# GadGadGad/Convolutional-KAN-for-Image-Classification

Measured on AMD Instinct MI355X. Metric: images/sec fwd+bwd KAN-VGG11 3x32x32 bs=256/GPU, higher is better.
Workload: dtype f32

## Files before the change

### convolutional-kan-for-image-classification_amd/csrc/kan_internal.h

```cpp
#pragma once
#include <type_traits>
#include "kanconv.h"

int kan_fail_msg(const char* fmt, const char* a);
int kan_raise_lds_limit(const void* kernel, int bytes);

enum : int {
    FAST_GENERIC = 0,
    FAST_BSPLINE_SILU = 1,
    FAST_BSPLINE_GELU = 2,
    FAST_RBF8 = 3,
    FAST_CHEBY5 = 4,
    FAST_CHEBY4 = 5,
    FAST_POLY4 = 6,
    FAST_POLY3 = 7,
    FAST_RBF5 = 8,
    FAST_RELU8 = 9,
    FAST_GRAM4 = 10,
    FAST_POLY1 = 11,
    FAST_LAST = 11
};
enum : unsigned {
    ON_TAP_MAJOR = 1u << 0,
    ON_BIG_TILES = 1u << 1,
// ... 22 lines not shown
        case FAST_CHEBY5: return {KAN_BASIS_CHEBY, 5, false, false, false, 16, ON_TAP_MAJOR | ON_BIG_TILES | ON_BAND_FWD | ON_BAND_BWD_WEIGHT};
        case FAST_CHEBY4: return {KAN_BASIS_CHEBY, 4, false, false, false, 16, ON_TAP_MAJOR | ON_HALO_FWD | ON_BAND_FWD};
        case FAST_POLY4: return {KAN_BASIS_POLY, 5, true, true, false, 16, ON_TAP_MAJOR | ON_BIG_TILES | ON_HALO_FWD | ON_BAND_FWD};
        case FAST_POLY3: return {KAN_BASIS_POLY, 4, true, true, false, 16, ON_TAP_MAJOR};
        case FAST_POLY1: return {KAN_BASIS_POLY, 2, true, true, false, 16, ON_TAP_MAJOR};
        case FAST_RELU8: return {KAN_BASIS_RELU, 9, true, false, false, 16, ON_HALO_FWD | ON_HALO_BWD_WEIGHT | ON_EXPANDED_FWD | ON_EXPANDED};
        case FAST_GRAM4: return {KAN_BASIS_GRAM, 5, true, false, false, 16, ON_HALO_FWD | ON_HALO_BWD_WEIGHT | ON_EXPANDED};
        default: return {-1, 0, false, true, true, 0, 0};
    }
}
constexpr int fast_kind(int f) { return fast_spec(f).kind; }
constexpr int fast_planes(int f) { return fast_spec(f).planes; }
constexpr bool fast_has(int f, unsigned routes) { return (fast_spec(f).routes & routes) == routes && f != FAST_GENERIC; }

template <int V> using IC = std::integral_constant<int, V>;
template <unsigned ROUTES, int F = 1, class Fn>
bool dispatch_fast(int f, Fn&& fn) {
    if constexpr (F > FAST_LAST) {
        return false;
    } else {
        if constexpr (fast_has(F, ROUTES)) {
            if (f == F) { fn(IC<F>{}); return true; }
        }
        return dispatch_fast<ROUTES, F + 1>(f, fn);
    }
}
template <int V, int... REST, class Fn>
void pick(int v, Fn&& fn) {
    if constexpr (sizeof...(REST) == 0) fn(IC<V>{});
    else if (v == V) fn(IC<V>{});
    else pick<REST...>(v, fn);
}
template <class Fn>
void dispatch_kind(int kind, Fn&& fn) {
    pick<KAN_BASIS_BSPLINE, KAN_BASIS_RBF, KAN_BASIS_POLY, KAN_BASIS_FOURIER, KAN_BASIS_RELU, KAN_BASIS_GRAM, KAN_BASIS_CHEBY>(kind, fn);
}

#define KAN_BAND_MAX_TAPS 128
#define KAN_BAND_MAX_PHASES 16
typedef struct KanBandCfg {
    int ok;
    int fast, P, NG, NPLE, NPS;
    int NGR;
    int WO, MO, WP, TO, TP, NT;
    int tiles_o, tiles_p;
    int n_phase, n_taps, n_steps;
    int HC, span_r, OR0, OC0;
    int cells;
    int slots;
    int TS;
    int lds_bytes, wgs_per_cu;
    int fwd_splits;
    int bw_ok, bw_WR, bw_NI, bw_NT, bw_tiles_o, bw_row_tiles, bw_TPI, bw_ptiles, bw_cells, bw_slots, bw_lds_bytes, bw_splits;
    unsigned short bw_ph_rt0[KAN_BAND_MAX_PHASES + 1];
    unsigned char ph_a[KAN_BAND_MAX_PHASES], ph_b[KAN_BAND_MAX_PHASES];
    short ph_tap0[KAN_BAND_MAX_PHASES + 1];
    unsigned short tap_shift[KAN_BAND_MAX_TAPS];
    unsigned short tap_rt[KAN_BAND_MAX_TAPS];
    short tap_step[KAN_BAND_MAX_TAPS], tap_nt[KAN_BAND_MAX_TAPS];
} KanBandCfg;

void kan_band_cfg(const KanGeom* g, const KanBasis* b, int fast, KanBandCfg* cfg);
int kan_band_bwd_weight_launch(const float* dz, const float* x, const float* xn, float* dwp, const KanGeom* g, const KanBasis* b,
                               const KanBandCfg* cfg, int splits, long long slab_elems, void* stream);
int kan_band_fwd_launch(const float* x, const float* xn, const float* wp, float* z, const KanGeom* g, const KanBasis* b,
                        const KanBandCfg* cfg, int splits, long long slab_elems, void* stream);

constexpr int DW_T = 9;
constexpr int DW_MAX_TP = 96;

enum class Route { TAP_MAJOR, DW, BAND, HALO, EXPANDED };

struct FwdCfg { int TO, TP, tiles_o, tiles_p, chunks, splits, slots; };
struct BdCfg { int CH, tiles_c, tiles_p, n_ob, Opad32, chunks, splits; };
struct BwCfg { int TR, TO, tiles_r, tiles_o, chunks, splits, slots; };
struct BwHaloCfg { int R, nimg, spb, n_bands, tiles_r, tiles_o, splits, bands_per_split; };

struct ConvPlan {
    KanPlan pub;
    int fast;
    Route fwd, bwd_data, bwd_weight;
    bool pm_fwd, pm_bwd_data, pm_bwd_weight;
    bool rowblk_bwd_data;
    bool pmdma_xcd, pm_lpt, pm_xcd;
    FwdCfg fc;
    BdCfg bd;
    BwCfg bw;
    BwHaloCfg bwh;
    KanBandCfg band;
};
int plan_conv(const KanGeom* g, const KanBasis* b, ConvPlan* cp);

int live_taps_out(const KanGeom* g, int hw);
int live_taps_in(const KanGeom* g, int hw);
int live_positions_for_tap(const KanGeom* g, int tap);
int balance_tiles(const int* weight, int n, unsigned short* idx);
```

### convolutional-kan-for-image-classification_amd/csrc/kan_plan.hip

```cpp
#include <hip/hip_runtime.h>
#include <cstdio>
#include <cstdlib>
#include <cstring>
#include "kanconv.h"
#include "kan_device.h"
#include "kan_common.h"
#include "kan_internal.h"

namespace {

int fail(const char* msg) { return kan_fail_msg("%s", msg); }

int check(const KanGeom* g, const KanBasis* b) {
    if (!g || !b) return fail("null geometry/basis");
    if (g->groups < 0 || g->groups > 65535) return fail("groups out of range");
    if (g->B <= 0 || g->C <= 0 || g->O <= 0 || g->H <= 0 || g->W <= 0 || g->Ho <= 0 || g->Wo <= 0) return fail("non-positive dimension");
    if (g->kh <= 0 || g->kw <= 0 || g->sh <= 0 || g->sw <= 0 || g->dh <= 0 || g->dw <= 0 || g->ph < 0 || g->pw < 0) return fail("bad conv parameters");
    if (g->kh > 255 || g->kw > 255 || g->C > 65535) return fail("kernel size / channel count out of supported range");
    if ((g->H + 2 * g->ph - g->dh * (g->kh - 1) - 1) / g->sh + 1 != g->Ho || (g->W + 2 * g->pw - g->dw * (g->kw - 1) - 1) / g->sw + 1 != g->Wo)
        return fail("Ho/Wo inconsistent with H/W, kernel, stride, padding, dilation");
    if ((long long)g->B * g->Ho * g->Wo >= (1ll << 31) || (long long)g->B * g->H * g->W >= (1ll << 31)) return fail("pixel count exceeds int32");
    if ((long long)g->B * g->x_bstride * 4 >= (1ll << 31) || (long long)g->B * g->y_bstride * 4 >= (1ll << 31))
        return fail("activation tensors must be smaller than 2 GiB (32-bit buffer offsets)");
    if (g->x_bstride < (long long)ngroups(g) * g->C * g->H * g->W || g->y_bstride < (long long)ngroups(g) * g->O * g->Ho * g->Wo)
// ... 248 lines not shown
    return n;
}

int balance_tiles(const int* weight, int n, unsigned short* idx) {
    if (n < 2 || n > PERM_MAX) return 0;
    int order[PERM_MAX];
    for (int i = 0; i < n; ++i) order[i] = i;
    for (int i = 1; i < n; ++i) {
        int v = order[i], j = i;
        while (j > 0 && weight[order[j - 1]] < weight[v]) { order[j] = order[j - 1]; --j; }
        order[j] = v;
    }
    for (int r = 0; r < n; ++r) {
        const int depth = r / 8, k = r % 8, bin = (depth & 1) ? 7 - k : k;
        int slot = depth * 8 + bin;
        if (slot >= n) slot = r;
        idx[slot] = (unsigned short)order[r];
    }
    bool seen[PERM_MAX] = {false};
    for (int i = 0; i < n; ++i) { if (idx[i] >= n || seen[idx[i]]) return 0; seen[idx[i]] = true; }
    return n;
}

int plan_conv(const KanGeom* g, const KanBasis* b, ConvPlan* cp) {
    if (int rc = check(g, b)) return rc;
    ConvPlan& c = *cp;
    KanPlan* pl = &c.pub;
    const int T = g->kh * g->kw, G = ngroups(g), f = fast_variant(b);
    c.fast = f;
    const bool pm_shape = pmdma_fwd_shape(g, f);
    c.pm_fwd = want_pix_major(g, b, PM_FWD, pm_shape);
    c.pm_bwd_data = want_pix_major(g, b, PM_BWD_DATA, false);
    const bool want_pm_bw = want_pix_major(g, b, PM_BWD_WEIGHT, false);
    const bool dw = dw_direct(g, b);
    const bool halo = halo_fwd(g, b, f, c.pm_fwd);
    c.band.ok = c.band.bw_ok = 0;
    const bool band = band_fwd(g, b, f, dw, c.pm_fwd, halo, &c.band);
    const bool pmdma_fwd = pm_shape && c.pm_fwd;
    const bool pmdma_bw = pmdma_bwd_weight(g, b, f, want_pm_bw);
    const bool halo_bw = halo_bwd_weight(g, f, pmdma_bw);
    c.pm_bwd_weight = want_pm_bw && !halo_bw;
    const bool band_bw = band && c.band.bw_ok && !want_pm_bw && !tuning_off("KAN_BAND_BW");
    c.rowblk_bwd_data = rowblk_bwd_data(g, f, c.pm_bwd_data);
    c.pmdma_xcd = tuning_on("KAN_PMDMA_XCD");
    c.pm_lpt = !tuning_off("KAN_PM_LPT");
    c.pm_xcd = !tuning_off("KAN_PM_XCD");
    c.fwd = dw ? Route::DW : band ? Route::BAND : halo ? Route::HALO : pmdma_fwd ? Route::EXPANDED : Route::TAP_MAJOR;
    c.bwd_data = dw ? Route::DW : Route::TAP_MAJOR;
    c.bwd_weight = dw ? Route::DW : band_bw ? Route::BAND : halo_bw ? Route::HALO : pmdma_bw ? Route::EXPANDED : Route::TAP_MAJOR;
    pl->P = b->n_basis + (b->act != KAN_ACT_NONE);
    pl->K = g->C * T * pl->P;
    {
        int i18 = 18 / pl->P, i16 = 16 / pl->P;
        if (i18 > 4) i18 = 4;
        if (i16 > 4) i16 = 4;
        const bool use18 = (long long)i18 * pl->P * 16 > (long long)i16 * pl->P * 18;
        pl->KC = use18 ? 18 : 16;
        pl->IPC = use18 ? i18 : i16;
        if (pl->P >= 10 && pl->P <= 12) { pl->KC = 12; pl->IPC = 1; }
        if (halo) { pl->KC = 2 * pl->P; pl->IPC = 2; }
    }
    pl->Kpad = ceil_div(g->C * T, pl->IPC) * pl->KC;
    if (band) { pl->KC = c.band.NPLE; pl->IPC = c.band.NG; pl->Kpad = c.band.n_steps * c.band.NPLE; }
    pl->Opad = round_up(g->O, 64);
    pl->packed_weight_bytes = (long long)G * pl->Kpad * pl->Opad * 4;
    c.bd = bd_cfg(g, *pl);
    pl->bwd_data_weight_bytes = (long long)G * T * c.bd.Opad32 * c.bd.tiles_c * 128 * 4;
    pl->fwd_slab_elems = (long long)g->B * g->y_bstride;
    pl->bwd_data_slab_elems = (long long)g->B * g->x_bstride;
    pl->bwd_weight_slab_elems = (long long)G * pl->K * pl->Opad;
    const bool big = big_tiles(f, *pl);
    c.fc = fwd_cfg(g, *pl, big, c.pm_fwd, halo);
    c.bw = bw_cfg(g, *pl, big, c.pm_bwd_weight);
    if (halo_bw) c.bwh = bw_halo_cfg(g, *pl);
    pl->fwd_splits = band ? c.band.fwd_splits : c.fc.splits;
    pl->bwd_data_splits = c.bd.splits;
    pl->bwd_weight_splits = halo_bw ? c.bwh.splits : c.bw.splits;
    if (band_bw) {
        pl->bwd_weight_splits = c.band.bw_splits;
        pl->bwd_weight_slab_elems = (long long)G * pl->Kpad * pl->Opad;
    }
    pl->fwd_target = pl->bwd_data_target = pl->bwd_weight_target = 0;
    const bool rowblk_fwd = halo && g->H == 4 && g->W == 4 && c.fc.TO == 256;
    if (dw) {
        pl->fwd_splits = pl->bwd_data_splits = 1;
        pl->bwd_weight_splits = dw_weight_chunks(g);
        pl->bwd_data_weight_bytes = pl->packed_weight_bytes;
        c.pm_fwd = c.pm_bwd_data = c.pm_bwd_weight = false;
    }
    if (c.pm_fwd) {
        LiveClass cls[16]; const int plane = g->Ho * g->Wo;
        const long long tiles_per_pos = (long long)ceil_div(g->B, c.fc.TP) * c.fc.tiles_o * G;
        for (int hw = 0; hw < plane; ++hw) cls[hw] = LiveClass{tiles_per_pos, live_taps_out(g, hw) * ceil_div(g->C, pl->IPC)};
        pl->fwd_target = pick_target_steps(cls, plane, 8, 4.0 * g->B * g->O * g->Ho * g->Wo * G, &pl->fwd_splits, c.fc.slots);
    }
    if (c.pm_bwd_weight) {
        LiveClass cw[32];
        const long long tiles_per_tap = (long long)ceil_div((long long)g->C * pl->P, c.bw.TR) * c.bw.tiles_o * G;
        for (int tap = 0; tap < T; ++tap) cw[tap] = LiveClass{tiles_per_tap, live_positions_for_tap(g, tap) * ceil_div(g->B, 16)};
        pl->bwd_weight_target = pick_target_steps(cw, T, 16, 4.0 * pl->K * pl->Opad * G, &pl->bwd_weight_splits, c.bw.slots);
    }
    if (c.pm_bwd_data) {
        LiveClass cls[16]; const int plane = g->H * g->W;
        const long long tiles_per_pos = (long long)ceil_div(g->B, 128) * c.bd.tiles_c * G;
        for (int hw = 0; hw < plane; ++hw) cls[hw] = LiveClass{tiles_per_pos, live_taps_in(g, hw) * c.bd.n_ob};
        pl->bwd_data_target = pick_target_steps(cls, plane, 8, 4.0 * g->B * g->C * g->H * g->W * G, &pl->bwd_data_splits);
    }
    pl->fwd_halo = c.fwd == Route::HALO;
    pl->fwd_band = c.fwd == Route::BAND;
    pl->fwd_expanded = c.fwd == Route::EXPANDED;
    pl->bwd_weight_halo = c.bwd_weight == Route::HALO;
    pl->bwd_weight_band = c.bwd_weight == Route::BAND;
    pl->bwd_weight_expanded = c.bwd_weight == Route::EXPANDED;
    pl->x_pm_wanted = (c.pm_fwd && c.fwd != Route::EXPANDED) || (c.pm_bwd_weight && c.bwd_weight != Route::EXPANDED);
    pl->dz_pm_wanted = c.pm_bwd_data || c.pm_bwd_weight;
    pl->e_pm_wanted = pl->fwd_expanded || pl->bwd_weight_expanded;
    pl->e_pm_elems = pl->e_pm_wanted ? (long long)G * g->C * g->H * g->W * pl->P * g->B + 256 : 0;
    pl->row_blocks = (rowblk_fwd ? 1 : 0) | (c.rowblk_bwd_data ? 2 : 0);
    return 0;
}
```

### convolutional-kan-for-image-classification_amd/csrc/kanconv.hip

```cpp
#include <hip/hip_runtime.h>
#include <cstdio>
#include <cstdlib>
#include <cstring>
#include <cmath>
#include <cstdint>
#include <mutex>
#include <type_traits>
#include <vector>
#include "kanconv.h"
#include "kan_device.h"

#include "kan_common.h"
#include "kan_internal.h"

namespace {


thread_local char g_err[512] = "";
int fail(const char* fmt, const char* a = "") {
    snprintf(g_err, sizeof(g_err), fmt, a);
    return -1;
}
}
int kan_fail_msg(const char* fmt, const char* a) { return fail(fmt, a); }
// ... 328 lines not shown
        }
    };

    f32x16 acc[2][2];
#pragma unroll
    for (int a = 0; a < 2; ++a)
#pragma unroll
        for (int b = 0; b < 2; ++b)
#pragma unroll
            for (int r = 0; r < 16; ++r) acc[a][b][r] = 0.f;

    int ch0 = blk.z * chunks_per_split;
    int ch1 = min(n_chunks, ch0 + chunks_per_split);
    unsigned tapmask = 0xffffffffu;
    if (g.pix_major) {
        tapmask = 0;
        const int hwA = px_tile0 / g.B, hwB = min(px_tile0 + TP - 1, Mtot - 1) / g.B;
        for (int hw = hwA; hw <= hwB; ++hw)
            for (int tap = 0; tap < T; ++tap) tapmask |= (tap_alive_out(g, hw, tap) ? 1u : 0u) << tap;
        auto seg = [&](int tap) { return (tap * g.C + IPC - 1) / IPC; };
        const int L = live_step_count(tapmask, T, n_chunks, seg);
        const int S = min((int)gridDim.z, max(1, (L + chunks_per_split - 1) / chunks_per_split));
        if (blk.z >= S) { ch0 = ch1 = n_chunks; }
        else {
            ch0 = blk.z == 0 ? 0 : live_step_pos(tapmask, T, n_chunks, (int)((long long)L * blk.z / S), seg);
            ch1 = blk.z == S - 1 ? n_chunks : live_step_pos(tapmask, T, n_chunks, (int)((long long)L * (blk.z + 1) / S), seg);
        }
    }
    auto next_live = [&](int ch) -> int {
        if (!g.pix_major) return ch;
        while (ch < ch1) {
            const int tapA = (ch * IPC) / g.C, tapB = min(ch * IPC + IPC - 1, NI - 1) / g.C;
            if (((tapmask >> tapA) | (tapmask >> tapB)) & 1u) return ch;
            ch = max(ch + 1, ((tapB + 1) * g.C) / IPC);
        }
        return ch1;
    };
    int ch = next_live(ch0);
    if (ch < ch1) issue(ch, 0);
    __syncthreads();

    const int ao = w_o * 64 + (lane & 31), bp = w_p * 64 + (lane & 31), kh2 = lane >> 5;
    for (int cur = 0; ch < ch1; cur ^= 1) {
        stage(cur);
        asm volatile("s_waitcnt vmcnt(0)" ::: "memory");
        __syncthreads();
        ch = next_live(ch + 1);
        if (ch < ch1) issue(ch, cur ^ 1);
        const float* cW = sW + cur * (KC * TO);
        const float* cE = sE + cur * (KC * TP);
        const unsigned aw = lds_addr(cW + kh2 * TO + ao), ae = lds_addr(cE + kh2 * TP + bp);
        KAN_MFMA_STEP(KC / 2, aw, TO, ae, TP);
    }

    float* zs = z + (size_t)blk.z * slab_elems;
#pragma unroll
    for (int ni = 0; ni < 2; ++ni) {
        const int px = px_tile0 + w_p * 64 + ni * 32 + (lane & 31);
        if (px >= Mtot) continue;
        int b, hw;
        if (g.pix_major) { hw = px / g.B; b = px - hw * g.B; }
        else { b = px / HoWo; hw = px - b * HoWo; }
        float* zb = zs + (size_t)b * g.ybs + hw;
#pragma unroll
        for (int mi = 0; mi < 2; ++mi) {
#pragma unroll
            for (int r = 0; r < 16; ++r) {
                const int o = o_tile0 + w_o * 64 + mi * 32 + mfma_row(r, lane);
                if (o < g.O) zb[(size_t)o * HoWo] = acc[mi][ni][r];
            }
        }
    }
}

#define LDS_READ4H(r0, r1, r2, r3, addrA, addrB0, addrB1, oA0, oA1, oB)                                                 \
    asm volatile("ds_read_b32 %0, %4 offset:%7\n\tds_read_b32 %1, %4 offset:%8\n\tds_read_b32 %2, %5 offset:%9\n\tds_read_b32 %3, %6 offset:%9" \
                 : "=&v"(r0), "=&v"(r1), "=&v"(r2), "=&v"(r3) : "v"(addrA), "v"(addrB0), "v"(addrB1), "n"(oA0), "n"(oA1), "n"(oB) : "memory")

#define LDS_READ3H(r0, r1, r2, addrA, addrB, oA0, oA1, oB)                                                               \
    asm volatile("ds_read_b32 %0, %3 offset:%5\n\tds_read_b32 %1, %3 offset:%6\n\tds_read_b32 %2, %4 offset:%7"         \
                 : "=&v"(r0), "=&v"(r1), "=&v"(r2) : "v"(addrA), "v"(addrB), "n"(oA0), "n"(oA1), "n"(oB) : "memory")
#define LDS_WAIT3(r0, r1, r2, N) asm volatile("s_waitcnt lgkmcnt(" #N ")" : "+v"(r0), "+v"(r1), "+v"(r2) :: "memory")

template <int FAST, int WO, int W, int R, int NIMG>
__global__ __launch_bounds__(WO * 2 * 64, ((WO > 2 && !(R * W == 16 && NIMG * W == 32)) ? 2 : 4)) void k_conv_fwd_halo(
    const float* __restrict__ x, const float* __restrict__ wp, float* __restrict__ z, DevGeom g, DevBasis bs, int Opad,
    int n_pairs, int pairs_per_split, long long slab_elems, unsigned x_bytes, int tiles_o) {
    constexpr int TO = WO * 64, TP = 128, NT = WO * 2 * 64, NW = WO * 2, P = fast_planes(FAST), KC = 2 * P, T = 9;
    constexpr int KIND = fast_kind(FAST);
    constexpr int HW_ = W + 2, HIMG = (R + 2) * HW_, HALO = NIMG * HIMG;
    constexpr int RPI = 256 / TO, NQ = (KC + RPI - 1) / RPI;
    static_assert(NIMG * R * W == TP && HALO % 2 == 0, "tile shape");
    constexpr bool ROWBLK = (R * W == 16 && NIMG * W == 32 && WO == 4);
    __shared__ __attribute__((aligned(16))) float sW[2 * KC * TO];
    __shared__ float sH[2 * P * HALO];
    __shared__ float sTab[KAN_MAX_TABLE];
    __shared__ float sDump[NT];

    const int tid = threadIdx.x, lane = tid & 63;
    const int wave = __builtin_amdgcn_readfirstlane(tid >> 6);
    const int w_o = ROWBLK ? (wave & 3) : (wave >> 1), w_p = ROWBLK ? (wave >> 2) : (wave & 1);
    const int HoWo = g.Ho * g.Wo, HW = g.H * g.W, Mtot = g.B * HoWo;
    const BlockId blk = xcd_block_order(true);
    const int grp = blk.y / tiles_o;
    const int px_tile0 = blk.x * TP, o_tile0 = (blk.y - grp * tiles_o) * TO;
    x += (size_t)grp * g.C * HW;
    z += (size_t)grp * g.O * HoWo;
    wp += (size_t)grp * n_pairs * (T * KC) * Opad;

    if (tid < KAN_MAX_TABLE) sTab[tid] = bs.tab[tid];
    for (int i = tid; i < 2 * P * HALO; i += NT) sH[i] = 0.f;

    const int b0 = px_tile0 / HoWo, h0 = (px_tile0 - b0 * HoWo) / W;
    constexpr int NCELL = 2 * HALO, CPT = (NCELL + NT - 1) / NT;
    int c_src[CPT], c_dst[CPT], c_ch[CPT]; unsigned c_ok = 0;
#pragma unroll
    for (int k = 0; k < CPT; ++k) {
        const int idx = tid + k * NT;
        const int ch = idx / HALO, cell = idx - ch * HALO;
        const int img = cell / HIMG, rc = cell - img * HIMG, hr = rc / HW_, hc = rc - hr * HW_;
        const int b = b0 + img, h = h0 - 1 + hr, w = hc - 1;
        const bool ok = idx < NCELL && b < g.B && (unsigned)h < (unsigned)g.H && (unsigned)w < (unsigned)W;
        c_src[k] = b * (int)g.xbs + ch * HW + h * W + w;
        c_dst[k] = ch * (P * HALO) + cell;
        c_ch[k] = ch;
        c_ok |= (ok ? 1u : 0u) << k;
    }
    const kan_rsrc x_rs = make_rsrc(x, x_bytes);

    const int kh2 = lane >> 5;
    unsigned vb[2];
#pragma unroll
    for (int q = 0; q < 2; ++q) {
        const int n = w_p * 64 + q * 32 + (lane & 31);
        int img = n / (R * W), rem = n - img * (R * W), row = rem / W, col = rem - row * W;
        if (ROWBLK) { row = n / (NIMG * W); rem = n - row * (NIMG * W); img = rem / W; col = rem - img * W; }
        vb[q] = lds_addr(sH + kh2 * (P * HALO) + img * HIMG + (row + 1) * HW_ + (col + 1));
    }
    const int ao = w_o * 64 + (lane & 31);
    const unsigned wlane = (unsigned)((lane / (TO / 4)) * Opad + (lane % (TO / 4)) * 4) * 4u;
    const int wv = wave;

    auto issue_w = [&](int step, int buf) {
        const char* wsrc = (const char*)(wp + (size_t)step * KC * Opad + o_tile0);
        float* dW = sW + buf * (KC * TO);
#pragma unroll
        for (int j = 0; j < (NQ + NW - 1) / NW; ++j) {
            const int q = j * NW + wv;
            if (q < NQ) {
                if (KC % RPI == 0 || q * RPI + (int)(lane / (TO / 4)) < KC)
                    glds16((const float*)(wsrc + (size_t)q * RPI * Opad * 4 + wlane), dW + q * 256);
            }
        }
    };

    f32x16 acc[2][2];
#pragma unroll
    for (int a = 0; a < 2; ++a)
#pragma unroll
        for (int b = 0; b < 2; ++b)
#pragma unroll
            for (int r = 0; r < 16; ++r) acc[a][b][r] = 0.f;

    const int cp0 = blk.z * pairs_per_split, cp1 = min(n_pairs, cp0 + pairs_per_split);
    int buf = 0;
    float xv[CPT];
    auto load_pair = [&](int cp) {
#pragma unroll
        for (int k = 0; k < CPT; ++k)
            xv[k] = buf_load(x_rs, ((c_ok >> k) & 1u) ? (unsigned)(c_src[k] + 2 * cp * HW) * 4u : KAN_OOB);
    };
    if (cp0 < cp1) { issue_w(cp0 * T, 0); load_pair(cp0); }
    __syncthreads();
    for (int cp = cp0; cp < cp1; ++cp) {
        __syncthreads();
#pragma unroll
        for (int k = 0; k < CPT; ++k)
            if ((c_ok >> k) & 1u) stage_unit<KIND, FAST>(bs, sTab, true, xv[k], xv[k], sH + c_dst[k], HALO, sDump + tid, 2 * cp + c_ch[k]);
#pragma unroll 1
        for (int tap = 0; tap < T; ++tap) {
            asm volatile("s_waitcnt vmcnt(0)" ::: "memory");
            __syncthreads();
            const int nxt = cp * T + tap + 1;
            if (nxt < cp1 * T) issue_w(nxt, buf ^ 1);
            if (tap == 4 && cp + 1 < cp1) load_pair(cp + 1);
            const int r = tap / 3, t = tap - r * 3;
            const unsigned sh = (unsigned)(((r - 1) * HW_ + (t - 1)) * 4);
            const unsigned aw = lds_addr(sW + buf * (KC * TO) + kh2 * TO + ao), ab0 = vb[0] + sh, ab1 = vb[1] + sh;
            float fa[2][2], fb[2][2];
            const int dead = !ROWBLK ? -1 : (r == 0 && w_p == 0) ? 0 : (r == 2 && w_p == 1) ? 1 : -1;
            const bool live0 = dead != 0, live1 = dead != 1;
            LDS_READ4H(fa[0][0], fa[0][1], fb[0][0], fb[0][1], aw, ab0, ab1, 0, 32 * 4, 0);
#pragma unroll
            for (int kk = 0; kk < P; ++kk) {
                const int c_ = kk & 1, n_ = c_ ^ 1;
                if (kk + 1 < P) {
                    LDS_READ4H(fa[n_][0], fa[n_][1], fb[n_][0], fb[n_][1], aw, ab0, ab1, (2 * (kk + 1)) * TO * 4, (2 * (kk + 1)) * TO * 4 + 128,
                               (kk + 1) * HALO * 4);
                    LDS_WAIT4(fa[c_][0], fa[c_][1], fb[c_][0], fb[c_][1], 4);
                } else {
                    LDS_WAIT4(fa[c_][0], fa[c_][1], fb[c_][0], fb[c_][1], 0);
                }
                if (!ROWBLK || live0) {
                    acc[0][0] = MFMA32(fa[c_][0], fb[c_][0], acc[0][0]);
                    acc[1][0] = MFMA32(fa[c_][1], fb[c_][0], acc[1][0]);
                }
                if (!ROWBLK || live1) {
                    acc[0][1] = MFMA32(fa[c_][0], fb[c_][1], acc[0][1]);
                    acc[1][1] = MFMA32(fa[c_][1], fb[c_][1], acc[1][1]);
                }
            }
            buf ^= 1;
        }
    }

    float* zs = z + (size_t)blk.z * slab_elems;
#pragma unroll
    for (int ni = 0; ni < 2; ++ni) {
        int px = px_tile0 + w_p * 64 + ni * 32 + (lane & 31);
        if (ROWBLK) {
            const int l = lane & 31;
            px = px_tile0 + (l >> 2) * (R * W) + (w_p * 2 + ni) * W + (l & 3);
        }
        if (px >= Mtot) continue;
        const int b = px / HoWo, hw = px - b * HoWo;
        float* zb = zs + (size_t)b * g.ybs + hw;
#pragma unroll
        for (int mi = 0; mi < 2; ++mi) {
#pragma unroll
            for (int r = 0; r < 16; ++r) {
                const int o = o_tile0 + w_o * 64 + mi * 32 + mfma_row(r, lane);
                if (o < g.O) zb[(size_t)o * HoWo] = acc[mi][ni][r];
            }
        }
    }
}

template <int M>
__device__ __forceinline__ void wave_reduce_scatter(float (&v)[M], int lane, int& idx, float& tot) {
    int base = 0;
    int m = M;
#pragma unroll
    for (int off = 32; off >= 1; off >>= 1) {
        if (m > 1) {
            const int h = m / 2;
            const bool up = (lane & off) != 0;
#pragma unroll
            for (int i = 0; i < M / 2; ++i) {
                if (i < h) {
                    const float keep = up ? v[h + i] : v[i], send = up ? v[i] : v[h + i];
                    v[i] = keep + __shfl_xor(send, off, 64);
                }
            }
            base += up ? h : 0;
            m = h;
        } else {
            v[0] += __shfl_xor(v[0], off, 64);
        }
    }
    idx = base; tot = v[0];
}

template <int KIND, int FAST, int RB = 0>
__global__ __launch_bounds__(256, 4) void k_conv_bwd_data(
    const float* __restrict__ dz, const float* __restrict__ x, const float* __restrict__ xn, const float* __restrict__ wd,
    float* __restrict__ dx, float* __restrict__ dxn, DevGeom g, DevBasis bs, int CH, int n_ct, int n_ob, int Opad16,
    int n_chunks, int chunks_per_split, long long slab_elems, unsigned dz_bytes, TilePerm perm, float* __restrict__ dpar) {
    constexpr int TP = 128, KD = 16, NT = 256;
    __shared__ __attribute__((aligned(16))) float smem[2 * 2 * KD * 128];
    __shared__ float sTab[KAN_MAX_TABLE];

    const int tid = threadIdx.x, lane = tid & 63;
    const int wave = __builtin_amdgcn_readfirstlane(tid >> 6);
    const int w_r = wave >> 1, w_p = wave & 1;
    const int HoWo = g.Ho * g.Wo, HW = g.H * g.W, P = bs.P;
    const int Min = g.B * HW;
    const BlockId blk = xcd_block_order(false);
    const int grp = blk.y / n_ct;
    const int px_tile0 = (perm.n ? (int)perm.idx[blk.x] : blk.x) * TP, ct = blk.y - grp * n_ct;
    const int ncol = n_ct * 128;
    const int pxl = (wave & 1) * 64 + lane, ol0 = wave >> 1;
    const bool idle_rows = (ct * 2 + w_r) * CH >= g.C;
    {
        const size_t xo = (size_t)grp * g.C * HW;
        x += xo; xn += xo; dx += xo; if (dxn) dxn += xo;
        dz += (size_t)grp * g.O * HoWo * (g.pix_major ? g.B : 1);
        wd += (size_t)grp * (g.kh * g.kw) * Opad16 * ncol;
    }

    if (tid < KAN_MAX_TABLE) sTab[tid] = bs.tab[tid];
    const int my_px = px_tile0 + (RB ? ((pxl >> 2) & 7) * 16 + (pxl >> 5) * 4 + (pxl & 3) : pxl);
    const bool pv = my_px < Min;
    int pb, ph_, pw_;
    {
        int hw;
        if (g.pix_major) { hw = my_px / g.B; pb = my_px - hw * g.B; }
        else { pb = my_px / HW; hw = my_px - pb * HW; }
        ph_ = hw / g.W; pw_ = hw - ph_ * g.W;
    }
// ... 1744 lines not shown
    ConvPlan cp;
    if (plan_conv(g, b, &cp)) return 0;
    if ((long long)g->O * g->C * (b->n_basis + 1) * g->kh * g->kw >= (1ll << 31)) return 0;
    return (!pack_needs_clear(g, cp.pub) && cp.fwd != Route::DW && ngroups(g) == 1) ? 1 : 0;
}

int kan_pack_weights_cached(const float* w_base, const float* w_basis, float* wp, float* wd, const KanGeom* g, const KanBasis* b,
                            unsigned long long* ring, int cur, int force, int sample_stride, void* stream) {
    static_assert(KAN_FP_WORDS == 3 * FP_LANES, "ring size");
    if (!ring || cur < 0 || cur > 2 || sample_stride < 1) return fail("bad fingerprint ring arguments");
    if (!kan_pack_cacheable(g, b)) return fail("cached packing is not offered for this geometry (kan_pack_cacheable)");
    const int hb = b->act != KAN_ACT_NONE;
    if ((hb && !w_base) || !w_basis) return fail("null weight pointer");
    if (((size_t)w_basis & 15) || (hb && ((size_t)w_base & 15))) return fail("cached packing needs 16-byte aligned weight tensors");
    const int T = g->kh * g->kw;
    const long long na = hb ? (long long)g->O * g->C * T : 0, nbs = (long long)g->O * g->C * b->n_basis * T;
    const long long groups4 = ((na + 3) / 4 + (nbs + 3) / 4 + sample_stride - 1) / sample_stride;
    long long blocks = (groups4 + 256 * 8 - 1) / (256 * 8); if (blocks > 4096) blocks = 4096; if (blocks < 1) blocks = 1;
    hipLaunchKernelGGL(k_fingerprint, dim3((unsigned)blocks), dim3(256), 0, (hipStream_t)stream, hb ? w_base : w_basis, (unsigned)na, w_basis,
                       (unsigned)nbs, (unsigned)sample_stride, ring, cur);
    if (int rc = launch_ok("fingerprint")) return rc;
    return pack_weights_impl(w_base, w_basis, wp, wd, g, b, force ? nullptr : ring, cur, stream);
}

int kan_unpack_wgrad(const float* dwp, float* dw_base, float* dw_basis, const KanGeom* g, const KanBasis* b, void* stream) {
    ConvPlan cp;
    if (int rc = plan_conv(g, b, &cp)) return rc;
    const KanPlan& pl = cp.pub;
    const int hb = b->act != KAN_ACT_NONE;
    if ((hb && !dw_base) || !dw_basis || !dwp) return fail("null weight-gradient pointer");
    hipStream_t st = (hipStream_t)stream;
    const int T = g->kh * g->kw, G = ngroups(g);
    const long long dwp_gs = (long long)(pl.bwd_weight_band ? pl.Kpad : pl.K) * pl.Opad;
    PackGeo q = pack_geo(g, b, cp, true);
    int n_slabs = pl.bwd_weight_splits;
    if (n_slabs >= 32) {
        hipLaunchKernelGGL(k_fold_slabs, dim3(ceil_div(pl.bwd_weight_slab_elems, 64)), dim3(256), 0, st, const_cast<float*>(dwp), n_slabs,
                           pl.bwd_weight_slab_elems, pl.bwd_weight_slab_elems);
        n_slabs = 1;
    }
    const int nb_base = hb ? ceil_div(g->C * T, 32) : 0;
    dim3 grid(nb_base + ceil_div(g->C * b->n_basis * T, 32), ceil_div(g->O, 32), G);
    hipLaunchKernelGGL(k_unpack, grid, dim3(256), 0, st, dwp, dw_base, dw_basis, q, nb_base, n_slabs, pl.bwd_weight_slab_elems, dwp_gs);
    return launch_ok("unpack");
}

int kan_position_major(const float* src, float* dst, int B, int Cn, int HW, long long bstride, void* stream) {
    if (!src || !dst || B < 1 || Cn < 1 || HW < 1) return fail("bad position_major arguments");
    dim3 grid(ceil_div((long long)Cn * HW, 32), ceil_div(B, 32));
    hipLaunchKernelGGL(k_position_major, grid, dim3(256), 0, (hipStream_t)stream, src, dst, B, Cn * HW, bstride);
    return launch_ok("position_major");
}

int kan_conv_fwd(const float* x, const float* xn, const float* wp, float* z, const KanGeom* g, const KanBasis* b, const float* x_pm,
                 void* stream) {
    ConvPlan cp;
    if (int rc = plan_conv(g, b, &cp)) return rc;
    const KanPlan& pl = cp.pub;
    if (!x || !xn || !wp || !z) return fail("null tensor pointer");
    if ((b->kind == KAN_BASIS_RELU || b->kind == KAN_BASIS_GRAM) && !b->chan_table) return fail("ReLU / Gram bases need their device parameter table (chan_table)");
    hipStream_t st = (hipStream_t)stream;
    if (cp.fwd == Route::DW) {
        DevGeom dgd = dev_geom(g); DevBasis dbd = dev_basis(b);
        dim3 grid(ceil_div((long long)g->B * g->Ho * g->Wo, 256), ngroups(g));
        dispatch_kind(b->kind, [&](auto kind) {
            hipLaunchKernelGGL((k_dw_fwd<decltype(kind)::value>), grid, dim3(256), 0, st, x, xn, wp, z, dgd, dbd, pl.Opad, pl.IPC, pl.KC, pl.Kpad);
        });
        return launch_ok("dw_fwd");
    }
    if (cp.fwd == Route::BAND) {
        if (x != xn && !fast_spec(cp.fast).xn_fwd) return fail("this basis / activation pair runs on single-input kernels: pass xn == x");
        return kan_band_fwd_launch(x, xn, wp, z, g, b, &cp.band, pl.fwd_splits, pl.fwd_slab_elems, stream);
    }
    const FwdCfg& c = cp.fc;
    if ((long long)c.tiles_o * ngroups(g) > 65535) return fail("groups * output tiles exceed the grid limit");
    const unsigned x_bytes = (unsigned)((long long)g->B * g->x_bstride * 4);
    if (cp.fwd == Route::HALO) {
        if (x != xn) return fail("internal: halo forward kernel needs a single input tensor");
        DevGeom dgh = dev_geom(g); DevBasis dbh = dev_basis(b);
        const int n_pairs = g->C / 2, pps = ceil_div(n_pairs, pl.fwd_splits);
        dim3 gridh(c.tiles_p, c.tiles_o * ngroups(g), pl.fwd_splits);
        dispatch_fast<ON_HALO_FWD>(cp.fast, [&](auto fv) {
            constexpr int F = decltype(fv)::value;
            auto launch = [&](auto wo, auto w, auto r, auto nimg) {
                constexpr int WOV = decltype(wo)::value;
                hipLaunchKernelGGL((k_conv_fwd_halo<F, WOV, decltype(w)::value, decltype(r)::value, decltype(nimg)::value>), gridh, dim3(WOV * 128), 0,
                                   st, x, wp, z, dgh, dbh, pl.Opad, n_pairs, pps, pl.fwd_slab_elems, x_bytes, c.tiles_o);
            };
            auto planes = [&](auto wo) {
                if (g->W == 32) launch(wo, IC<32>{}, IC<4>{}, IC<1>{});
                else if (g->W == 16) launch(wo, IC<16>{}, IC<8>{}, IC<1>{});
                else if (g->W == 8) launch(wo, IC<8>{}, IC<8>{}, IC<2>{});
                else launch(wo, IC<4>{}, IC<4>{}, IC<8>{});
            };
            if constexpr (fast_has(F, ON_BIG_TILES)) {
                if (c.TO == 256) return planes(IC<4>{});
            }
            planes(IC<2>{});
        });
        return launch_ok("conv_fwd_halo");
    }
    DevGeom dg = dev_geom(g);
    dg.pix_major = (x_pm && x == xn && cp.pm_fwd) ? 1 : 0;
    if (dg.pix_major) { x = x_pm; xn = x_pm; }
    DevBasis db = dev_basis(b);
    dim3 grid(c.tiles_p, c.tiles_o * ngroups(g), pl.fwd_splits);
    const int cps = dg.pix_major ? pl.fwd_target : ceil_div(c.chunks, pl.fwd_splits);
    TilePerm perm; perm.n = 0;
    if (dg.pix_major) perm = tile_perm(c.tiles_p, [&](int t) {
        const int hw = (int)(((long long)t * c.TP) / g->B);
        return ceil_div(live_taps_out(g, hw < g->Ho * g->Wo ? hw : 0) * ceil_div(g->C, pl.IPC), cps > 0 ? cps : 1);
    });
    if (x != xn && !fast_spec(cp.fast).xn_fwd)
        return fail("this basis / activation pair runs on single-input kernels: pass xn == x");
    auto launch = [&](auto kind, auto fast, auto wo, auto kc) {
        constexpr int WO = decltype(wo)::value;
        hipLaunchKernelGGL((k_conv_fwd<decltype(kind)::value, decltype(fast)::value, WO, 2, decltype(kc)::value>), grid, dim3(WO * 2 * 64), 0, st,
                           x, xn, wp, z, dg, db, pl.Opad, pl.IPC, c.chunks, cps, pl.fwd_slab_elems, x_bytes, perm, c.tiles_o);
    };
    const bool fast = dispatch_fast<ON_TAP_MAJOR>(cp.fast, [&](auto fv) {
        constexpr int F = decltype(fv)::value;
        if constexpr (fast_has(F, ON_BIG_TILES)) {
            if (c.TO == 256) return launch(IC<fast_kind(F)>{}, fv, IC<4>{}, IC<fast_spec(F).kc>{});
        }
        if (c.TO == 128) launch(IC<fast_kind(F)>{}, fv, IC<2>{}, IC<fast_spec(F).kc>{});
        else launch(IC<fast_kind(F)>{}, fv, IC<1>{}, IC<fast_spec(F).kc>{});
    });
    if (!fast) dispatch_kind(b->kind, [&](auto kind) {
        pick<18, 12, 16>(pl.KC, [&](auto kc) {
            if (c.TO == 128) launch(kind, IC<FAST_GENERIC>{}, IC<2>{}, kc);
            else launch(kind, IC<FAST_GENERIC>{}, IC<1>{}, kc);
        });
    });
    return launch_ok("conv_fwd");
}

static int conv_bwd_data_impl(const float* dz, const float* x, const float* xn, const float* wd, float* dx, float* dxn, float* dpar,
                              const KanGeom* g, const KanBasis* b, const float* dz_pm, void* stream);

int kan_conv_bwd_data(const float* dz, const float* x, const float* xn, const float* wd, float* dx, float* dxn,
                      const KanGeom* g, const KanBasis* b, const float* dz_pm, void* stream) {
    return conv_bwd_data_impl(dz, x, xn, wd, dx, dxn, nullptr, g, b, dz_pm, stream);
}

int kan_conv_bwd_data_params(const float* dz, const float* x, const float* xn, const float* wd, float* dx, float* dxn, float* dparams,
                             const KanGeom* g, const KanBasis* b, const float* dz_pm, void* stream) {
    if (!dparams) return fail("null dparams");
    if (b && b->kind != KAN_BASIS_RELU && b->kind != KAN_BASIS_GRAM) return fail("kan_conv_bwd_data_params: only the ReLU-KAN and GRAM bases accumulate parameter gradients in this launch");
    return conv_bwd_data_impl(dz, x, xn, wd, dx, dxn, dparams, g, b, dz_pm, stream);
}

static int conv_bwd_data_impl(const float* dz, const float* x, const float* xn, const float* wd, float* dx, float* dxn, float* dpar,
                              const KanGeom* g, const KanBasis* b, const float* dz_pm, void* stream) {
    ConvPlan cp;
    if (int rc = plan_conv(g, b, &cp)) return rc;
    const KanPlan& pl = cp.pub;
    if (dpar && cp.bwd_data == Route::DW) return fail("kan_conv_bwd_data_params: depthwise layers take the weight-gradient route");
    if (!dz || !x || !xn || !wd || !dx) return fail("null tensor pointer");
    if ((b->kind == KAN_BASIS_RELU || b->kind == KAN_BASIS_GRAM) && !b->chan_table) return fail("ReLU / Gram bases need their device parameter table (chan_table)");
    if (!dxn && x != xn) return fail("dxn is required when xn != x");
    hipStream_t st = (hipStream_t)stream;
    if (cp.bwd_data == Route::DW) {
        DevGeom dgd = dev_geom(g); DevBasis dbd = dev_basis(b);
        dim3 grid(ceil_div((long long)g->B * g->H * g->W, 256), ngroups(g));
        dispatch_kind(b->kind, [&](auto kind) {
            hipLaunchKernelGGL((k_dw_bwd_data<decltype(kind)::value>), grid, dim3(256), 0, st, dz, x, xn, wd, dx, dxn, dgd, dbd, pl.Opad, pl.IPC, pl.KC, pl.Kpad);
        });
        return launch_ok("dw_bwd_data");
    }
    const BdCfg& c = cp.bd;
    DevGeom dg = dev_geom(g);
    dg.pix_major = (dz_pm && cp.pm_bwd_data) ? 1 : 0;
    if (dg.pix_major) dz = dz_pm;
    DevBasis db = dev_basis(b);
    if ((long long)c.tiles_c * ngroups(g) > 65535) return fail("groups * channel tiles exceed the grid limit");
    dim3 grid(c.tiles_p, c.tiles_c * ngroups(g), pl.bwd_data_splits);
// ... 320 lines not shown
```

### convolutional-kan-for-image-classification_amd/ops.py

```python
from __future__ import annotations

import contextlib
import ctypes as C
import os
import weakref
from collections import OrderedDict
from dataclasses import dataclass
from functools import lru_cache
from typing import List, Optional, Sequence, Tuple

import torch

from . import _lib as L


@dataclass(frozen=True)
class ConvSpec:
    kind: int
    n_basis: int
    order: int
    act: int
    p0: float
    p1: float
    table: Tuple[float, ...]
# ... 41 lines not shown
def _plan_key(spec: ConvSpec, shape, Og: int) -> tuple:
    B, Ct, H, W = shape
    return (spec, B, Ct // spec.groups, H, W, Og, Ct, Og * spec.groups)


def _with_phases(basis: L.KanBasis, phases: Optional[torch.Tensor], mode: int = 0) -> L.KanBasis:
    if phases is None:
        return basis
    b = L.KanBasis.from_buffer_copy(basis)
    b.chan_table, b.order = phases.data_ptr(), mode
    return b


def _ptr(t: Optional[torch.Tensor], offset: int = 0) -> C.c_void_p:
    if t is None:
        return C.c_void_p(0)
    return C.c_void_p(t.data_ptr() + 4 * offset)


def _stream(t: torch.Tensor) -> C.c_void_p:
    return C.c_void_p(torch.cuda.current_stream(t.device).cuda_stream)


def _require(t: torch.Tensor, name: str) -> torch.Tensor:
    if not t.is_cuda:
        raise L.KanConvError(f"{name} is on {t.device}: this path runs only on a ROCm device (MI355X); there is no CPU fallback")
    if t.dtype != torch.float32:
        raise L.KanConvError(f"{name} must be float32, got {t.dtype}")
    return t.contiguous()


def _split_weights(spec: ConvSpec, weights: Sequence[torch.Tensor]):
    G = spec.groups
    if spec.has_base:
        return list(weights[:G]), list(weights[G:2 * G])
    return [None] * G, list(weights[:G])


PROFILE: Optional[list] = None


@dataclass
class KernelSample:
    name: str
    flops: float
    executed: float
    layer: str
    start: "torch.cuda.Event"
    end: "torch.cuda.Event"


def _launch(sample, t: torch.Tensor, fn) -> None:
    name, flops, executed, layer = sample
    if PROFILE is None:
        L.check(fn(), name)
        return
    e0, e1 = torch.cuda.Event(enable_timing=True), torch.cuda.Event(enable_timing=True)
    stream = torch.cuda.current_stream(t.device)
    e0.record(stream)
    L.check(fn(), name)
    e1.record(stream)
    PROFILE.append(KernelSample(name, flops, executed, layer, e0, e1))


def _conv_flops(geom, plan) -> float:
    return 2.0 * geom.B * geom.O * geom.Ho * geom.Wo * geom.C * plan.P * geom.kh * geom.kw * max(1, geom.groups)


@lru_cache(maxsize=256)
def _live_fraction(which: str, H: int, W: int, Ho: int, Wo: int, kh: int, kw: int, sh: int, sw: int, ph: int, pw: int, dh: int, dw: int) -> float:
    live = 0
    for ho in range(Ho):
        for wo in range(Wo):
            for r in range(kh):
                for t in range(kw):
                    hi, wi = ho * sh - ph + r * dh, wo * sw - pw + t * dw
                    live += 0 <= hi < H and 0 <= wi < W
    return live / float(Ho * Wo * kh * kw)


_ROW_BLOCK_BIT = {"fwd": 1, "bwd_data": 2, "bwd_weight": 0}


def _executed_flops(geom, plan, which: str) -> float:
    target = {"fwd": plan.fwd_target, "bwd_data": plan.bwd_data_target, "bwd_weight": plan.bwd_weight_target}[which]
    dense = _conv_flops(geom, plan)
    if target <= 0:
        if plan.row_blocks & _ROW_BLOCK_BIT[which]:
            return dense * (5.0 / 6.0)
        return dense
    g = geom
    return dense * _live_fraction(which, g.H, g.W, g.Ho, g.Wo, g.kh, g.kw, g.sh, g.sw, g.ph, g.pw, g.dh, g.dw)


def _layer_tag(geom) -> str:
    return f"{geom.C * max(1, geom.groups)}->{geom.O * max(1, geom.groups)}@{geom.H}x{geom.W} k{geom.kh}x{geom.kw}"


def _sample(which: str, geom, plan, pm: bool, two: bool = False, expanded: bool = False):
    tile = "128" if plan.Opad % 128 == 0 else "64"
    if which == "bwd_data":
        name = "k_conv_bwd_data"
    elif expanded:
        name = f"k_conv_{which}_pmdma/o{tile}"
    elif plan.fwd_band if which == "fwd" else plan.bwd_weight_band:
        name = f"k_band_{which}/o" + ("128" if plan.Opad % 128 == 0 else "192" if plan.Opad == 192 else "64")
    else:
        halo = plan.fwd_halo if which == "fwd" else (plan.bwd_weight_halo and not two)
        name = f"k_conv_{which}{'_halo' if halo else ''}/o{tile}"
    skips = expanded or pm or bool(plan.row_blocks & _ROW_BLOCK_BIT[which])
    dense = _conv_flops(geom, plan)
    return name, dense, _executed_flops(geom, plan, which) if skips else dense, _layer_tag(geom)


def _position_major(t: torch.Tensor, ch_off: int, Cn: int) -> torch.Tensor:
    B, Ct, H, W = t.shape
    out = torch.empty(Cn * H * W * B, device=t.device, dtype=torch.float32)
    L.check(L.load().kan_position_major(_ptr(t, ch_off * H * W), _ptr(out), B, Cn, H * W, Ct * H * W, _stream(t)), "kan_position_major")
    return out


def _stack(ws: Sequence[Optional[torch.Tensor]]) -> Optional[torch.Tensor]:
    if ws[0] is None:
        return None
    return ws[0].unsqueeze(0) if len(ws) == 1 else torch.stack(list(ws))


_PACKED: "OrderedDict[tuple, PackedWeights]" = OrderedDict()
_PACK_CACHE_MAX = int(os.environ.get("KAN_PACK_CACHE", "256"))
_PACK_CACHE_BYTES = int(os.environ.get("KAN_PACK_CACHE_BYTES", str(16 << 30)))
_PACK_SAMPLE = max(1, int(os.environ.get("KAN_PACK_SAMPLE", "1")))
_PACK_VERIFY_EVERY = int(os.environ.get("KAN_PACK_VERIFY_EVERY", "16"))
_EPOCH = 0
PACK_STATS = {"calls": 0, "forced": 0, "skipped": 0}


_ALWAYS_PACK = False


@contextlib.contextmanager
def always_pack():
    global _ALWAYS_PACK
    prev, _ALWAYS_PACK = _ALWAYS_PACK, True
    try:
        yield
    finally:
        _ALWAYS_PACK = prev


_SPLIT_INFERENCE = False
_SPLIT_CACHE: "OrderedDict" = OrderedDict()


@contextlib.contextmanager
def split_precision_inference():
    global _SPLIT_INFERENCE
    prev, _SPLIT_INFERENCE = _SPLIT_INFERENCE, True
    try:
        yield
    finally:
        _SPLIT_INFERENCE = prev


def _split_stage(spec: ConvSpec, x: torch.Tensor, w_base, w_basis):
    if spec.groups != 1 or not spec.has_base or x.dim() != 4:
        return None
    lib = L.load()
    wb, ws = w_base[0], w_basis[0]
    geom, basis, _ = _plan_cached(*_plan_key(spec, x.shape, ws.shape[0]))
    if not lib.kan_split_supported(C.byref(geom), C.byref(basis)):
        return None
    key = (wb.data_ptr(), ws.data_ptr(), x.device.index)
    stamps = (_owner(wb)._version, _owner(ws)._version, _EPOCH)
    ent = _SPLIT_CACHE.get(key)
# ... 532 lines not shown
```

Baseline: 17280.

## Add quadrant-ordered 4x4 halo forward tile skipping dead border taps per pixel

Adds a QUAD variant of the halo forward kernel for 4x4 layers: each 128-pixel tile covers one 2x2 spatial quadrant across 32 images, with a 3x3 halo per image. Each pixel column gets a per-tap liveness mask, so MFMAs for padded taps are skipped wherever they fall outside the image. The old row-block scheme only skipped 1/6 of taps. Output stores become float2 writes. The cost is a different halo layout and store pattern, plus alignment guards on z and the strides. The path is used only when B%32==0 and can be disabled through an environment variable.

After: 17480 (median of 6 runs). 1.01x the previous value.

```diff
diff --git a/convolutional-kan-for-image-classification_amd/csrc/kan_internal.h b/convolutional-kan-for-image-classification_amd/csrc/kan_internal.h
--- a/convolutional-kan-for-image-classification_amd/csrc/kan_internal.h
+++ b/convolutional-kan-for-image-classification_amd/csrc/kan_internal.h
@@ -128,6 +128,7 @@
     Route fwd, bwd_data, bwd_weight;
     bool pm_fwd, pm_bwd_data, pm_bwd_weight;
     bool rowblk_bwd_data;
+    bool quad_fwd;
     bool pmdma_xcd, pm_lpt, pm_xcd;
     FwdCfg fc;
     BdCfg bd;
diff --git a/convolutional-kan-for-image-classification_amd/csrc/kan_plan.hip b/convolutional-kan-for-image-classification_amd/csrc/kan_plan.hip
--- a/convolutional-kan-for-image-classification_amd/csrc/kan_plan.hip
+++ b/convolutional-kan-for-image-classification_amd/csrc/kan_plan.hip
@@ -354,6 +354,7 @@
     }
     pl->fwd_target = pl->bwd_data_target = pl->bwd_weight_target = 0;
     const bool rowblk_fwd = halo && g->H == 4 && g->W == 4 && c.fc.TO == 256;
+    c.quad_fwd = rowblk_fwd && g->B % 32 == 0 && !tuning_off("KAN_QUAD_FWD");
     if (dw) {
         pl->fwd_splits = pl->bwd_data_splits = 1;
         pl->bwd_weight_splits = dw_weight_chunks(g);
diff --git a/convolutional-kan-for-image-classification_amd/csrc/kanconv.hip b/convolutional-kan-for-image-classification_amd/csrc/kanconv.hip
--- a/convolutional-kan-for-image-classification_amd/csrc/kanconv.hip
+++ b/convolutional-kan-for-image-classification_amd/csrc/kanconv.hip
@@ -434,36 +434,40 @@
                  : "=&v"(r0), "=&v"(r1), "=&v"(r2) : "v"(addrA), "v"(addrB), "n"(oA0), "n"(oA1), "n"(oB) : "memory")
 #define LDS_WAIT3(r0, r1, r2, N) asm volatile("s_waitcnt lgkmcnt(" #N ")" : "+v"(r0), "+v"(r1), "+v"(r2) :: "memory")
 
-template <int FAST, int WO, int W, int R, int NIMG>
+template <int FAST, int WO, int W, int R, int NIMG, int QUAD = 0>
 __global__ __launch_bounds__(WO * 2 * 64, ((WO > 2 && !(R * W == 16 && NIMG * W == 32)) ? 2 : 4)) void k_conv_fwd_halo(
     const float* __restrict__ x, const float* __restrict__ wp, float* __restrict__ z, DevGeom g, DevBasis bs, int Opad,
     int n_pairs, int pairs_per_split, long long slab_elems, unsigned x_bytes, int tiles_o) {
     constexpr int TO = WO * 64, TP = 128, NT = WO * 2 * 64, NW = WO * 2, P = fast_planes(FAST), KC = 2 * P, T = 9;
     constexpr int KIND = fast_kind(FAST);
-    constexpr int HW_ = W + 2, HIMG = (R + 2) * HW_, HALO = NIMG * HIMG;
+    constexpr int HW_ = QUAD ? 3 : W + 2, HIMG = QUAD ? 9 : (R + 2) * HW_, HALO = (QUAD ? 32 : NIMG) * HIMG;
     constexpr int RPI = 256 / TO, NQ = (KC + RPI - 1) / RPI;
     static_assert(NIMG * R * W == TP && HALO % 2 == 0, "tile shape");
-    constexpr bool ROWBLK = (R * W == 16 && NIMG * W == 32 && WO == 4);
+    static_assert(!QUAD || (R * W == 16 && NIMG * W == 32 && WO == 4), "the quadrant order is a variant of the row-block tile");
+    constexpr bool ROWBLK = (R * W == 16 && NIMG * W == 32 && WO == 4) && !QUAD;
+    constexpr int HPAD = QUAD ? 4 : 0;
     __shared__ __attribute__((aligned(16))) float sW[2 * KC * TO];
-    __shared__ float sH[2 * P * HALO];
+    __shared__ float sH_[2 * P * HALO + 2 * HPAD];
+    float* const sH = sH_ + HPAD;
     __shared__ float sTab[KAN_MAX_TABLE];
     __shared__ float sDump[NT];
 
     const int tid = threadIdx.x, lane = tid & 63;
     const int wave = __builtin_amdgcn_readfirstlane(tid >> 6);
-    const int w_o = ROWBLK ? (wave & 3) : (wave >> 1), w_p = ROWBLK ? (wave >> 2) : (wave & 1);
+    const int w_o = (ROWBLK || QUAD) ? (wave & 3) : (wave >> 1), w_p = (ROWBLK || QUAD) ? (wave >> 2) : (wave & 1);
     const int HoWo = g.Ho * g.Wo, HW = g.H * g.W, Mtot = g.B * HoWo;
     const BlockId blk = xcd_block_order(true);
     const int grp = blk.y / tiles_o;
+    const int qh = (blk.x >> 1) & 1, qw = blk.x & 1;
     const int px_tile0 = blk.x * TP, o_tile0 = (blk.y - grp * tiles_o) * TO;
     x += (size_t)grp * g.C * HW;
     z += (size_t)grp * g.O * HoWo;
     wp += (size_t)grp * n_pairs * (T * KC) * Opad;
 
     if (tid < KAN_MAX_TABLE) sTab[tid] = bs.tab[tid];
-    for (int i = tid; i < 2 * P * HALO; i += NT) sH[i] = 0.f;
-
-    const int b0 = px_tile0 / HoWo, h0 = (px_tile0 - b0 * HoWo) / W;
+    for (int i = tid; i < 2 * P * HALO + 2 * HPAD; i += NT) sH_[i] = 0.f;
+
+    const int b0 = QUAD ? (blk.x >> 2) * 32 : px_tile0 / HoWo, h0 = QUAD ? 0 : (px_tile0 - b0 * HoWo) / W;
     constexpr int NCELL = 2 * HALO, CPT = (NCELL + NT - 1) / NT;
     int c_src[CPT], c_dst[CPT], c_ch[CPT]; unsigned c_ok = 0;
 #pragma unroll
@@ -471,7 +475,7 @@
         const int idx = tid + k * NT;
         const int ch = idx / HALO, cell = idx - ch * HALO;
         const int img = cell / HIMG, rc = cell - img * HIMG, hr = rc / HW_, hc = rc - hr * HW_;
-        const int b = b0 + img, h = h0 - 1 + hr, w = hc - 1;
+        const int b = b0 + img, h = QUAD ? qh + hr : h0 - 1 + hr, w = QUAD ? qw + hc : hc - 1;
         const bool ok = idx < NCELL && b < g.B && (unsigned)h < (unsigned)g.H && (unsigned)w < (unsigned)W;
         c_src[k] = b * (int)g.xbs + ch * HW + h * W + w;
         c_dst[k] = ch * (P * HALO) + cell;
@@ -482,11 +486,24 @@
 
     const int kh2 = lane >> 5;
     unsigned vb[2];
+    int q_hw[2] = {0, 0}; unsigned q_live[2] = {0x1ffu, 0x1ffu};
 #pragma unroll
     for (int q = 0; q < 2; ++q) {
         const int n = w_p * 64 + q * 32 + (lane & 31);
         int img = n / (R * W), rem = n - img * (R * W), row = rem / W, col = rem - row * W;
         if (ROWBLK) { row = n / (NIMG * W); rem = n - row * (NIMG * W); img = rem / W; col = rem - img * W; }
+        if (QUAD) {
+            const int h = 2 * qh + w_p, w = 2 * qw + q;
+            q_hw[q] = h * 4 + w;
+            unsigned m = 0;
+            for (int tap = 0; tap < 9; ++tap) {
+                const int r = tap / 3, t = tap - r * 3;
+                m |= (((unsigned)(h + r - 1) < 4u && (unsigned)(w + t - 1) < 4u) ? 1u : 0u) << tap;
+            }
+            q_live[q] = m;
+            vb[q] = lds_addr(sH + kh2 * (P * HALO) + (lane & 31) * HIMG + (h - qh) * HW_ + (w - qw));
+            continue;
+        }
         vb[q] = lds_addr(sH + kh2 * (P * HALO) + img * HIMG + (row + 1) * HW_ + (col + 1));
     }
     const int ao = w_o * 64 + (lane & 31);
@@ -541,7 +558,7 @@
             const unsigned aw = lds_addr(sW + buf * (KC * TO) + kh2 * TO + ao), ab0 = vb[0] + sh, ab1 = vb[1] + sh;
             float fa[2][2], fb[2][2];
             const int dead = !ROWBLK ? -1 : (r == 0 && w_p == 0) ? 0 : (r == 2 && w_p == 1) ? 1 : -1;
-            const bool live0 = dead != 0, live1 = dead != 1;
+            const bool live0 = QUAD ? ((q_live[0] >> tap) & 1u) != 0 : dead != 0, live1 = QUAD ? ((q_live[1] >> tap) & 1u) != 0 : dead != 1;
             LDS_READ4H(fa[0][0], fa[0][1], fb[0][0], fb[0][1], aw, ab0, ab1, 0, 32 * 4, 0);
 #pragma unroll
             for (int kk = 0; kk < P; ++kk) {
@@ -553,11 +570,11 @@
                 } else {
                     LDS_WAIT4(fa[c_][0], fa[c_][1], fb[c_][0], fb[c_][1], 0);
                 }
-                if (!ROWBLK || live0) {
+                if (!(ROWBLK || QUAD) || live0) {
                     acc[0][0] = MFMA32(fa[c_][0], fb[c_][0], acc[0][0]);
                     acc[1][0] = MFMA32(fa[c_][1], fb[c_][0], acc[1][0]);
                 }
-                if (!ROWBLK || live1) {
+                if (!(ROWBLK || QUAD) || live1) {
                     acc[0][1] = MFMA32(fa[c_][0], fb[c_][1], acc[0][1]);
                     acc[1][1] = MFMA32(fa[c_][1], fb[c_][1], acc[1][1]);
                 }
@@ -567,6 +584,18 @@
     }
 
     float* zs = z + (size_t)blk.z * slab_elems;
+    if (QUAD) {
+        float* zb = zs + (size_t)(b0 + (lane & 31)) * g.ybs + q_hw[0];
+#pragma unroll
+        for (int mi = 0; mi < 2; ++mi) {
+#pragma unroll
+            for (int r = 0; r < 16; ++r) {
+                const int o = o_tile0 + w_o * 64 + mi * 32 + mfma_row(r, lane);
+                if (o < g.O) *reinterpret_cast<float2*>(zb + (size_t)o * HoWo) = make_float2(acc[mi][0][r], acc[mi][1][r]);
+            }
+        }
+        return;
+    }
 #pragma unroll
     for (int ni = 0; ni < 2; ++ni) {
         int px = px_tile0 + w_p * 64 + ni * 32 + (lane & 31);
@@ -2477,16 +2506,20 @@
         dim3 gridh(c.tiles_p, c.tiles_o * ngroups(g), pl.fwd_splits);
         dispatch_fast<ON_HALO_FWD>(cp.fast, [&](auto fv) {
             constexpr int F = decltype(fv)::value;
-            auto launch = [&](auto wo, auto w, auto r, auto nimg) {
+            auto launch = [&](auto wo, auto w, auto r, auto nimg, auto quad) {
                 constexpr int WOV = decltype(wo)::value;
-                hipLaunchKernelGGL((k_conv_fwd_halo<F, WOV, decltype(w)::value, decltype(r)::value, decltype(nimg)::value>), gridh, dim3(WOV * 128), 0,
-                                   st, x, wp, z, dgh, dbh, pl.Opad, n_pairs, pps, pl.fwd_slab_elems, x_bytes, c.tiles_o);
+                hipLaunchKernelGGL((k_conv_fwd_halo<F, WOV, decltype(w)::value, decltype(r)::value, decltype(nimg)::value, decltype(quad)::value>), gridh,
+                                   dim3(WOV * 128), 0, st, x, wp, z, dgh, dbh, pl.Opad, n_pairs, pps, pl.fwd_slab_elems, x_bytes, c.tiles_o);
             };
             auto planes = [&](auto wo) {
-                if (g->W == 32) launch(wo, IC<32>{}, IC<4>{}, IC<1>{});
-                else if (g->W == 16) launch(wo, IC<16>{}, IC<8>{}, IC<1>{});
-                else if (g->W == 8) launch(wo, IC<8>{}, IC<8>{}, IC<2>{});
-                else launch(wo, IC<4>{}, IC<4>{}, IC<8>{});
+                if constexpr (decltype(wo)::value == 4) {
+                    if (g->W == 4 && cp.quad_fwd && ((uintptr_t)z & 7u) == 0 && (g->y_bstride & 1) == 0 && (pl.fwd_slab_elems & 1) == 0)
+                        return launch(wo, IC<4>{}, IC<4>{}, IC<8>{}, IC<1>{});
+                }
+                if (g->W == 32) launch(wo, IC<32>{}, IC<4>{}, IC<1>{}, IC<0>{});
+                else if (g->W == 16) launch(wo, IC<16>{}, IC<8>{}, IC<1>{}, IC<0>{});
+                else if (g->W == 8) launch(wo, IC<8>{}, IC<8>{}, IC<2>{}, IC<0>{});
+                else launch(wo, IC<4>{}, IC<4>{}, IC<8>{}, IC<0>{});
             };
             if constexpr (fast_has(F, ON_BIG_TILES)) {
                 if (c.TO == 256) return planes(IC<4>{});
diff --git a/convolutional-kan-for-image-classification_amd/ops.py b/convolutional-kan-for-image-classification_amd/ops.py
--- a/convolutional-kan-for-image-classification_amd/ops.py
+++ b/convolutional-kan-for-image-classification_amd/ops.py
@@ -147,14 +147,20 @@
 _ROW_BLOCK_BIT = {"fwd": 1, "bwd_data": 2, "bwd_weight": 0}
 
 
+def _quadrant_order(geom, plan, which: str) -> bool:
+    return which == "fwd" and bool(plan.row_blocks & 1) and geom.B % 32 == 0
+
+
 def _executed_flops(geom, plan, which: str) -> float:
     target = {"fwd": plan.fwd_target, "bwd_data": plan.bwd_data_target, "bwd_weight": plan.bwd_weight_target}[which]
     dense = _conv_flops(geom, plan)
+    g = geom
     if target <= 0:
+        if _quadrant_order(geom, plan, which):
+            return dense * _live_fraction(which, g.H, g.W, g.Ho, g.Wo, g.kh, g.kw, g.sh, g.sw, g.ph, g.pw, g.dh, g.dw)
         if plan.row_blocks & _ROW_BLOCK_BIT[which]:
             return dense * (5.0 / 6.0)
         return dense
-    g = geom
     return dense * _live_fraction(which, g.H, g.W, g.Ho, g.Wo, g.kh, g.kw, g.sh, g.sw, g.ph, g.pw, g.dh, g.dw)
 
 
```
